# DerrickXuNu/CoBEVT

Measured on AMD Instinct MI355X. Metric: bev_frames_per_sec, higher is better.
Workload: dtype bf16

## Files before the change

cobevt_amd/csrc/stem7x7.hip:

```cpp
#include "common.hpp"
#include "f32_matrix.hpp"

namespace cobevt {

struct StemParams {
    const float* in;
    const unsigned char* in_u8;
    const float* lut;
    const void* wgt;
    const float* bias;
    void* out;
    int N, H, W, Ho, Wo, Cout;
    int act;
    int tiles_y, tiles_x, tiles_n, ntiles;
};

__device__ __forceinline__ uint4 lds_read_2x8(const unsigned char* a) {
    typedef const volatile __attribute__((address_space(3))) unsigned long long* lds_u64_ptr;
    const unsigned long long lo = *(lds_u64_ptr)a, hi = *(lds_u64_ptr)(a + 8);
    return make_uint4((unsigned)lo, (unsigned)(lo >> 32), (unsigned)hi, (unsigned)(hi >> 32));
}

template <typename T> struct StemCfg {
    static constexpr int KB = Elem<T>::kBytes;
    static constexpr int STEPS_ROW = 48 * KB / 32;
    static constexpr int PIX = 12 * KB;
    static constexpr int PH = 11, PW = 19;
    static constexpr int PROW = (PW * PIX - 16 * PIX % 256 + 255) / 256 * 256 + 16 * PIX % 256;
    static constexpr int PATCH = (PH * PROW + 255) / 256 * 256;
    static constexpr int WROW = 192 * KB + 16;
    static constexpr int WBYTES = 64 * WROW;
    static constexpr int SROW = 64 * 4 + 16;
    static constexpr int STAGE = 128 * SROW;
    static constexpr int LDS = PATCH + WBYTES + STAGE;
};

template <typename T>
__global__ __launch_bounds__(256) void stem7x7_kernel(StemParams p) {
    using C = StemCfg<T>;
    constexpr int KB = C::KB;
    constexpr int NPIECE = C::PH * C::PW * 2 * 3;
    constexpr int P_IT = (NPIECE + 255) / 256;
    extern __shared__ __attribute__((aligned(16))) unsigned char smem[];
    unsigned char* patch = smem;
    unsigned char* wl = smem + C::PATCH;
    float* stage = (float*)(smem + C::PATCH + C::WBYTES);

    const int tid = threadIdx.x, lane = tid & 63, wave = tid >> 6;
    const int h = lane >> 5, ql = lane & 31;

    for (int i = tid; i < C::PATCH / 16; i += 256) ((uint4*)patch)[i] = make_uint4(0, 0, 0, 0);

    float2 preg[P_IT];
    auto decode = [&](int tile, int& img, int& oy0, int& ox0, int& n0) {
        const int tn = tile % p.tiles_n;
        int rest = tile / p.tiles_n;
        const int tx = rest % p.tiles_x; rest /= p.tiles_x;
        const int ty = rest % p.tiles_y;
        img = rest / p.tiles_y;
        oy0 = ty * 8; ox0 = tx * 16; n0 = tn * 64;
    };
    auto load_patch = [&](int tile) {
        int img, oy0, ox0, n0;
        decode(tile, img, oy0, ox0, n0);
#pragma unroll
        for (int it = 0; it < P_IT; ++it) {
            const int item = tid + it * 256;
            float2 v = make_float2(0.f, 0.f);
            if (item < NPIECE) {
                const int pc = item % 3, rest = item / 3;
                const int dy = rest & 1, pix = rest >> 1;
                const int py = pix / C::PW, px = pix - py * C::PW;
                const int iy = 2 * (oy0 - 2 + py) + dy, ix = 2 * (ox0 - 2 + px);
                if (iy >= 0 && iy < p.H && ix >= 0 && ix + 1 < p.W)
                    v = *(const float2*)(p.in + (((size_t)img * p.H + iy) * p.W + ix) * 3 + pc * 2);
            }
            preg[it] = v;
        }
    };
    auto store_patch = [&]() {
#pragma unroll
        for (int it = 0; it < P_IT; ++it) {
            const int item = tid + it * 256;
            if (item < NPIECE) {
                const int pc = item % 3, rest = item / 3;
                const int dy = rest & 1, pix = rest >> 1;
                const int py = pix / C::PW, px = pix - py * C::PW;
                unsigned char* dst = patch + py * C::PROW + px * C::PIX + (dy * 6 + pc * 2) * KB;
                if constexpr (Elem<T>::kIsBf16) *(uint32_t*)dst = pack_bf2(preg[it].x, preg[it].y);
                else *(float2*)dst = preg[it];
            }
        }
    };

    int img, oy0, ox0, n0;
    int tile = blockIdx.x;
    if (tile >= p.ntiles) return;
    decode(tile, img, oy0, ox0, n0);
    int n0_loaded = -1;
    auto load_weights = [&](int nb) {
        constexpr int PIECES = 16 * 16 * Elem<T>::kBytes / 16;
        constexpr int PPT = PIECES / 16;
        for (int i = tid; i < 64 * PIECES; i += 256) {
            const int row = i / PIECES, j = i - row * PIECES;
            const int tap = j / PPT, part = j - tap * PPT;
            uint4 v = make_uint4(0, 0, 0, 0);
            if (nb + row < p.Cout) v = *(const uint4*)((const unsigned char*)p.wgt + ((size_t)(nb + row) * PIECES + j) * 16);
            unsigned char* d = wl + row * C::WROW + ((tap >> 2) * 48 + (tap & 3) * 12) * KB + part * 16;
            if constexpr (Elem<T>::kIsBf16) {
                *(uint2*)d = make_uint2(v.x, v.y);
                if (part == 0) *(uint2*)(d + 8) = make_uint2(v.z, v.w);
            } else if (part < 3) {
                *(uint4*)d = v;
            }
        }
        n0_loaded = nb;
    };
    __syncthreads();
    load_patch(tile);
    load_weights(n0);

    const int abase = ((2 * wave + (ql >> 4)) * C::PROW) + (ql & 15) * C::PIX + h * 16;
    const int bbase = ql * C::WROW + h * 16;

    for (; tile < p.ntiles; tile += gridDim.x) {
        decode(tile, img, oy0, ox0, n0);
        store_patch();
        if (n0 != n0_loaded) { __syncthreads(); load_weights(n0); }
        __syncthreads();
        const int next = tile + gridDim.x;
        if (next < p.ntiles) load_patch(next);

        f32x16 acc[2];
#pragma unroll
        for (int b = 0; b < 2; ++b)
#pragma unroll
            for (int r = 0; r < 16; ++r) acc[b][r] = 0.f;
#pragma unroll
        for (int a = 0; a < 4; ++a) {
#pragma unroll
            for (int sub = 0; sub < C::STEPS_ROW; ++sub) {
                const unsigned char* pa = patch + abase + a * C::PROW + sub * 32;
                const unsigned char* pw = wl + bbase + a * 48 * KB + sub * 32;
                uint4 af;
                if constexpr (Elem<T>::kIsBf16) {
                    af = lds_read_2x8(pa);
                } else {
                    af = *(const uint4*)pa;
                }
                const uint4 b0 = *(const uint4*)pw;
                const uint4 b1 = *(const uint4*)(pw + 32 * C::WROW);
                mfma_kgroup<T, false>(af, b0, acc[0]);
                mfma_kgroup<T, false>(af, b1, acc[1]);
            }
        }
        constexpr int SR = C::SROW / 4;
#pragma unroll
        for (int b = 0; b < 2; ++b) {
            const int cl = b * 32 + ql;
            const float bias = (p.bias && n0 + cl < p.Cout) ? p.bias[n0 + cl] : 0.f;
#pragma unroll
            for (int r = 0; r < 16; ++r) {
                const int row = acc_row(r, lane);
                float v = acc[b][r] + bias;
                v = p.act == 1 ? fmaxf(v, 0.f) : v;
                stage[((2 * wave + (row >> 4)) * 16 + (row & 15)) * SR + cl] = v;
            }
        }
        __syncthreads();
        constexpr int CH = Elem<T>::kChunk;
        constexpr int CPP = 64 / CH;
        T* out = (T*)p.out;
        for (int item = tid; item < 128 * CPP; item += 256) {
            const int px = item / CPP, cj = item - px * CPP;
            const int oy = oy0 + (px >> 4), ox = ox0 + (px & 15), col = n0 + cj * CH;
            if (oy >= p.Ho || ox >= p.Wo || col >= p.Cout) continue;
            float v[8];
#pragma unroll
            for (int e = 0; e < CH; ++e) v[e] = stage[px * SR + cj * CH + e];
            const size_t o = (((size_t)img * p.Ho + oy) * p.Wo + ox) * p.Cout + col;
            if (col + CH <= p.Cout) *(uint4*)(out + o) = f32_to_chunk<T>(v);
            else for (int e = 0; e < CH && col + e < p.Cout; ++e) store_elem<T>(out, o + e, v[e]);
        }
        __syncthreads();
    }
}


#ifndef COBEVT_STEM_POOL_ROWS_BF16
#define COBEVT_STEM_POOL_ROWS_BF16 5
#endif
#ifndef COBEVT_STEM_POOL_ROWS_F32
#define COBEVT_STEM_POOL_ROWS_F32 3
#endif
#ifndef COBEVT_STEM_KNOCK
#define COBEVT_STEM_KNOCK 0
#endif

typedef short short2_t __attribute__((ext_vector_type(2)));
template <typename T> __device__ __forceinline__ uint32_t word_max(uint32_t a, uint32_t b) {
    if constexpr (Elem<T>::kIsBf16) {
        const short2_t r = __builtin_elementwise_max(__builtin_bit_cast(short2_t, a), __builtin_bit_cast(short2_t, b));
        return __builtin_bit_cast(uint32_t, r);
    } else {
        return (uint32_t)max((int)a, (int)b);
    }
}

template <typename T> struct StemPoolCfg {
    static constexpr int KB = Elem<T>::kBytes;
    static constexpr int STEPS_ROW = 48 * KB / 32;
    static constexpr int NS = 4 * STEPS_ROW;
    static constexpr int PIX = 12 * KB;
    static constexpr int ROWS = Elem<T>::kIsBf16 ? COBEVT_STEM_POOL_ROWS_BF16 : COBEVT_STEM_POOL_ROWS_F32;
    static constexpr int RH = 2 * ROWS + 1, RW = 17, RPIX = RH * RW;
    static constexpr int NPT = (RPIX + 31) / 32;
    static constexpr int NT = 64 * NPT * 2;
    static constexpr int PH = RH + 3, PW = RW + 3;
    static constexpr int PROW = (PW * PIX - RW * PIX % 256 + 255) / 256 * 256 + RW * PIX % 256;
    static constexpr int PATCH = (PH * PROW + 255) / 256 * 256;
    static constexpr int WROW = 192 * KB + 16;
    static constexpr int WBYTES = 64 * WROW;
    static constexpr int SROW = 64 * Elem<T>::kBytes + 16;
    static constexpr int STAGE = (RPIX * SROW + 255) / 256 * 256;
    static constexpr int LDS = PATCH + WBYTES + STAGE + 256;
    static constexpr int LDS_U8 = LDS + 3 * 256 * 4;
    static_assert(NT <= 1024, "stem_pool_kernel: region too large for one workgroup");
};

#ifdef COBEVT_STEM_TRACE
__device__ unsigned long long cobevt_stem_trace[16];
#define COBEVT_ST_MARK(i) do { if (blockIdx.x == 0 && threadIdx.x == 0 && tile == (int)blockIdx.x + 2 * (int)gridDim.x) cobevt_stem_trace[(i)] = __builtin_readcyclecounter(); } while (0)
#else
#define COBEVT_ST_MARK(i) do {} while (0)
#endif

template <typename T, bool U8 = false>
__global__ __launch_bounds__(StemPoolCfg<T>::NT) void stem_pool_kernel(StemParams p) {
    using C = StemPoolCfg<T>;
    constexpr int RW = C::RW, RPIX = C::RPIX, NT = C::NT, KB = C::KB;
    constexpr int NPIECE = C::PH * C::PW * 2 * 3;
    constexpr int P_IT = (NPIECE + NT - 1) / NT;
    extern __shared__ __attribute__((aligned(16))) unsigned char smem[];
    unsigned char* patch = smem;
    unsigned char* wl = smem + C::PATCH;
    unsigned char* stage = smem + C::PATCH + C::WBYTES;

    const int tid = threadIdx.x, lane = tid & 63, wave = tid >> 6;
    const int h = lane >> 5, ql = lane & 31;
    const int Hp = p.Ho / 2, Wp = p.Wo / 2;

    for (int i = tid; i < C::PATCH / 16; i += NT) ((uint4*)patch)[i] = make_uint4(0, 0, 0, 0);

    int pdst[P_IT], prow[P_IT], pxo[P_IT], pcol[P_IT];
    int plut[P_IT];
#pragma unroll
    for (int it = 0; it < P_IT; ++it) {
        const int item = tid + it * NT;
        pdst[it] = -1; prow[it] = 0; pxo[it] = 0; pcol[it] = 0; plut[it] = 0;
        if (item < NPIECE) {
            const int pc = item % 3, rest = item / 3;
            const int dy = rest & 1, pix = rest >> 1;
            const int py = pix / C::PW, px = pix - py * C::PW;
            pdst[it] = py * C::PROW + px * C::PIX + (dy * 6 + pc * 2) * KB;
            prow[it] = 2 * (py - 2) + dy;
            pxo[it] = 2 * (px - 2);
            pcol[it] = pxo[it] * 3 + pc * 2;
            plut[it] = ((pc * 2) % 3) | (((pc * 2 + 1) % 3) << 8);
        }
    }
    int poff[P_IT];
#pragma unroll
    for (int it = 0; it < P_IT; ++it) poff[it] = prow[it] * p.W * 3 + pcol[it];
    float2 preg[P_IT];
    unsigned int praw[P_IT];
    const float* lut_l = (const float*)(smem + C::LDS);
    auto decode = [&](int tile, int& img, int& py0, int& px0) {
        const int tx = tile % p.tiles_x;
        const int rest = tile / p.tiles_x;
        const int ty = rest % p.tiles_y;
        img = rest / p.tiles_y;
        py0 = ty * C::ROWS; px0 = tx * 8;
    };
    auto load_patch = [&](int tile) {
        int img, py0, px0;
        decode(tile, img, py0, px0);
        const int oy0 = 2 * py0 - 1, ox0 = 2 * px0 - 1;
        const size_t origin = ((size_t)img * p.H + 2 * oy0) * (size_t)p.W * 3 + 6 * ox0;
        const float* base = p.in + origin;
        const unsigned char* base8 = p.in_u8 + origin;
        const int ylo = -2 * oy0, yhi = p.H - 2 * oy0, xlo = -2 * ox0, xhi = p.W - 1 - 2 * ox0;
#pragma unroll
        for (int it = 0; it < P_IT; ++it) {
            const bool ok = (pdst[it] >= 0) & (prow[it] >= ylo) & (prow[it] < yhi) & (pxo[it] >= xlo) & (pxo[it] < xhi);
            if constexpr (U8) {
                unsigned int r = 0x10000u;
                if (!(COBEVT_STEM_KNOCK & 8) && ok) r = *(const unsigned short*)(base8 + poff[it]);
                praw[it] = r;
            } else {
                float2 v = make_float2(0.f, 0.f);
                if (!(COBEVT_STEM_KNOCK & 8) && ok) v = *(const float2*)(base + poff[it]);
                preg[it] = v;
            }
        }
    };
    auto store_patch = [&]() {
        if constexpr (U8) {
#pragma unroll
            for (int it = 0; it < P_IT; ++it) {
                const unsigned int r = praw[it];
                const float a = lut_l[(plut[it] & 0xff) * 256 + (r & 0xff)], b = lut_l[(plut[it] >> 8) * 256 + ((r >> 8) & 0xff)];
                preg[it] = (r >> 16) ? make_float2(0.f, 0.f) : make_float2(a, b);
            }
        }
#pragma unroll
        for (int it = 0; it < P_IT; ++it)
            if (pdst[it] >= 0) {
                unsigned char* dst = patch + pdst[it];
                if constexpr (Elem<T>::kIsBf16) *(uint32_t*)dst = pack_bf2(preg[it].x, preg[it].y);
                else if constexpr (kXSplit<T>) {
                    uint32_t hi, lo;
                    split_pair_staged(preg[it].x, preg[it].y, hi, lo);
                    unsigned char* pb = patch + (pdst[it] & ~15) + ((pdst[it] >> 1) & 4);
                    *(uint32_t*)pb = hi;
                    *(uint32_t*)(pb + 8) = lo;
                } else *(float2*)dst = preg[it];
            }
    };

    int tile = blockIdx.x;
    if (tile >= p.ntiles) return;
    if constexpr (U8) {
        float* l = (float*)(smem + C::LDS);
        for (int i = tid; i < 768; i += NT) l[i] = p.lut[i];
    }
    {
        load_patch(tile);
        constexpr int PIECES = 16 * 16 * KB / 16;
        constexpr int PPT = PIECES / 16;
        constexpr int W_IT = (64 * PIECES + NT - 1) / NT;
        uint4 wv[W_IT];
#pragma unroll
        for (int it = 0; it < W_IT; ++it) {
            const int i = tid + it * NT;
            const int row = i / PIECES, j = i - row * PIECES;
            wv[it] = *(const uint4*)((const unsigned char*)p.wgt + ((size_t)(row < p.Cout ? row : 0) * PIECES + (i < 64 * PIECES ? j : 0)) * 16);
        }
#pragma unroll
        for (int it = 0; it < W_IT; ++it) {
            const int i = tid + it * NT;
            const int row = i / PIECES, j = i - row * PIECES;
            const int tap = j / PPT, part = j - tap * PPT;
            if (i < 64 * PIECES) {
                const uint4 v = row < p.Cout ? wv[it] : make_uint4(0, 0, 0, 0);
                unsigned char* d = wl + row * C::WROW + ((tap >> 2) * 48 + (tap & 3) * 12) * KB + part * 16;
                if constexpr (Elem<T>::kIsBf16) {
                    *(uint2*)d = make_uint2(v.x, v.y);
                    if (part == 0) *(uint2*)(d + 8) = make_uint2(v.z, v.w);
                } else if (part < 3) {
                    *(uint4*)d = stage_w_piece<T>(v);
                }
            }
        }
    }

    const int chalf = wave & 1;
    const int rpix = (wave >> 1) * 32 + ql;
    const int rpc = rpix < RPIX ? rpix : RPIX - 1;
    const int ry = rpc / RW, rx = rpc - ry * RW;
    const int abase = ry * C::PROW + rx * C::PIX + h * 16;
    const int bbase = (chalf * 32 + ql) * C::WROW + h * 16;
    float* bias_l = (float*)(smem + C::PATCH + C::WBYTES + C::STAGE);
    if (tid < 64) bias_l[tid] = p.bias ? p.bias[tid] : 0.f;
    __syncthreads();

    constexpr int CH = Elem<T>::kChunk;
    constexpr int CPP = 64 / CH;
    static_assert((C::ROWS + 1) / 2 * 2 * 8 * CPP <= NT, "stem_pool_kernel: one pooled chunk per thread (rows in pairs)");
    uint4 pend = make_uint4(0, 0, 0, 0);
    T* pend_dst = nullptr;

    for (; tile < p.ntiles; tile += gridDim.x) {
        int img, py0, px0;
        decode(tile, img, py0, px0);
        const int oy0 = 2 * py0 - 1, ox0 = 2 * px0 - 1;
        COBEVT_ST_MARK(0);
        store_patch();
        if (pend_dst) *(uint4*)pend_dst = pend;
        __syncthreads();
        COBEVT_ST_MARK(1);
        const int next = tile + gridDim.x;
        if (next < p.ntiles) load_patch(next);
        COBEVT_ST_MARK(2);

        f32x16 acc;
#pragma unroll
        for (int r = 0; r < 16; ++r) acc[r] = 0.f;
        constexpr int NS = C::NS;
        constexpr int RS = 2;
        uint4 ra[RS], rb[RS];
        auto fetch = [&](int slot, int i) {
            const int a = i / C::STEPS_ROW, sub = i - a * C::STEPS_ROW;
            rb[slot] = *(const uint4*)(wl + bbase + a * 48 * KB + sub * 32);
            const unsigned char* pa = patch + abase + a * C::PROW + sub * 32;
            if constexpr (Elem<T>::kIsBf16) {
                ra[slot] = lds_read_2x8(pa);
            } else {
                ra[slot] = *(const uint4*)pa;
            }
        };
#pragma unroll
        for (int i = 0; i < RS - 1; ++i) fetch(i, i);
        __builtin_amdgcn_sched_barrier(0);
#pragma unroll
        for (int i = 0; i < NS; ++i) {
            if (i + RS - 1 < NS && !(COBEVT_STEM_KNOCK & 1)) fetch((i + RS - 1) % RS, i + RS - 1);
            if constexpr (COBEVT_STEM_KNOCK & 2) asm volatile("" :: "v"(rb[i % RS].x), "v"(rb[i % RS].y), "v"(rb[i % RS].z), "v"(rb[i % RS].w), "v"(ra[i % RS].x), "v"(ra[i % RS].y), "v"(ra[i % RS].z), "v"(ra[i % RS].w));
            else
            mfma_kgroup_staged<T>(rb[i % RS], ra[i % RS], acc);
            __builtin_amdgcn_sched_barrier(0);
        }
        COBEVT_ST_MARK(3);
        if (rpix < RPIX && !(COBEVT_STEM_KNOCK & 16)) {
            const int oy = oy0 + ry, ox = ox0 + rx;
            const bool inside = oy >= 0 && oy < p.Ho && ox >= 0 && ox < p.Wo;
            float4 bq[4];
#pragma unroll
            for (int k = 0; k < 4; ++k) bq[k] = *(const float4*)(bias_l + chalf * 32 + 8 * k + 4 * h);
            __builtin_amdgcn_sched_barrier(0);
#pragma unroll
            for (int k = 0; k < 4; ++k) {
                const int c0 = chalf * 32 + 8 * k + 4 * h;
                const float4 b = bq[k];
                float v[4] = {acc[4 * k] + b.x, acc[4 * k + 1] + b.y, acc[4 * k + 2] + b.z, acc[4 * k + 3] + b.w};
#pragma unroll
                for (int e = 0; e < 4; ++e) v[e] = inside ? fmaxf(v[e], 0.f) : 0.f;
                unsigned char* d = stage + rpix * C::SROW + c0 * Elem<T>::kBytes;
                if constexpr (Elem<T>::kIsBf16) *(uint2*)d = make_uint2(pack_bf2(v[0], v[1]), pack_bf2(v[2], v[3]));
                else *(float4*)d = make_float4(v[0], v[1], v[2], v[3]);
            }
        }
        COBEVT_ST_MARK(4);
        __syncthreads();
        COBEVT_ST_MARK(5);
        pend_dst = nullptr;
        int q_y, q_x, cj;
        if constexpr (Elem<T>::kIsBf16) {
            const int hw = tid >> 5, j = (tid >> 3) & 3, t = hw & 3;
            q_y = 2 * (hw >> 2) + (j & 1);
            q_x = j == 0 ? t : j == 1 ? ((t + 7) & 7) : j == 2 ? t + 4 : t + 3;
            cj = tid & 7;
        } else {
            const int q = tid / CPP;
            q_y = q >> 3; q_x = q & 7; cj = tid - q * CPP;
        }
        if (q_y < C::ROWS) {
            const int qy = q_y, qx = q_x;
            const int py = py0 + qy, px = px0 + qx;
            uint4 wv[9];
#pragma unroll
            for (int dy = 0; dy < 3; ++dy)
#pragma unroll
                for (int dx = 0; dx < 3; ++dx) {
                    wv[dy * 3 + dx] = *(const uint4*)(stage + ((2 * qy + dy) * RW + 2 * qx + dx) * C::SROW + cj * 16);
                    if constexpr (COBEVT_STEM_KNOCK & 4) wv[dy * 3 + dx] = make_uint4(dy, dx, dy, dx);
                }
            __builtin_amdgcn_sched_barrier(0);
            uint4 m = make_uint4(0, 0, 0, 0);
#pragma unroll
            for (int i = 0; i < 9; ++i) {
                m.x = word_max<T>(m.x, wv[i].x); m.y = word_max<T>(m.y, wv[i].y);
                m.z = word_max<T>(m.z, wv[i].z); m.w = word_max<T>(m.w, wv[i].w);
            }
            pend = m;
            if (py < Hp && px < Wp) pend_dst = (T*)p.out + (((size_t)img * Hp + py) * Wp + px) * 64 + cj * CH;
        }
        COBEVT_ST_MARK(6);
        __syncthreads();
        COBEVT_ST_MARK(7);
    }
    if (pend_dst) *(uint4*)pend_dst = pend;
}

}

using namespace cobevt;

extern "C" int cobevt_stem_conv7x7s2(const float* in, const void* wgt, const float* bias, void* out, const int* dims,
                                     hipStream_t stream) {
    if (!in || !wgt || !out || !dims) return COBEVT_ERR_ARG;
    StemParams p;
    const int dtype = dims[0];
    p.in = in; p.in_u8 = nullptr; p.lut = nullptr; p.wgt = wgt; p.bias = bias; p.out = out;
    p.N = dims[1]; p.H = dims[2]; p.W = dims[3]; p.Cout = dims[4]; p.act = dims[5];
    if (dtype != 0 && dtype != 1) return COBEVT_ERR_ARG;
    if (p.N < 1 || p.H < 2 || p.W < 2 || (p.H & 1) || (p.W & 1) || p.Cout < 1) return COBEVT_ERR_SHAPE;
    if (p.Cout % (dtype == 0 ? 8 : 4)) return COBEVT_ERR_SHAPE;
    p.Ho = p.H / 2; p.Wo = p.W / 2;
    p.tiles_y = (p.Ho + 7) / 8; p.tiles_x = (p.Wo + 15) / 16; p.tiles_n = (p.Cout + 63) / 64;
    const long nt = (long)p.N * p.tiles_y * p.tiles_x * p.tiles_n;
    if (nt > 0x7fffffffL) return COBEVT_ERR_SHAPE;
    p.ntiles = (int)nt;
    const size_t lds = dtype == 0 ? StemCfg<bf16_t>::LDS : StemCfg<float>::LDS;
    cobevt::allow_dynamic_lds<stem7x7_kernel<bf16_t>>((int)StemCfg<bf16_t>::LDS);
    cobevt::allow_dynamic_lds<stem7x7_kernel<float>>((int)StemCfg<float>::LDS);
    const int per_cu = dtype == 0 ? 2 : 1;
    const unsigned blocks = (unsigned)(nt < 256L * per_cu ? nt : 256L * per_cu);
    if (dtype == 0) hipLaunchKernelGGL(stem7x7_kernel<bf16_t>, dim3(blocks), dim3(256), lds, stream, p);
    else hipLaunchKernelGGL(stem7x7_kernel<float>, dim3(blocks), dim3(256), lds, stream, p);
    return cobevt::launch_status();
}

extern "C" int cobevt_stem_conv7x7s2_pool(const float* in, const void* wgt, const float* bias, void* out, const int* dims,
                                          hipStream_t stream) {
    if (!in || !wgt || !out || !dims) return COBEVT_ERR_ARG;
    StemParams p;
    const int dtype = dims[0];
    p.in = in; p.in_u8 = nullptr; p.lut = nullptr; p.wgt = wgt; p.bias = bias; p.out = out;
    p.N = dims[1]; p.H = dims[2]; p.W = dims[3]; p.Cout = 64; p.act = 1;
    if (dtype != 0 && dtype != 1) return COBEVT_ERR_ARG;
    if (p.N < 1 || p.H < 4 || p.W < 4 || (p.H & 3) || (p.W & 3)) return COBEVT_ERR_SHAPE;
    p.Ho = p.H / 2; p.Wo = p.W / 2;
    const int rows = dtype == 0 ? StemPoolCfg<bf16_t>::ROWS : StemPoolCfg<float>::ROWS;
    p.tiles_y = (p.Ho / 2 + rows - 1) / rows; p.tiles_x = (p.Wo / 2 + 7) / 8; p.tiles_n = 1;
    const long nt = (long)p.N * p.tiles_y * p.tiles_x;
    if (nt > 0x7fffffffL) return COBEVT_ERR_SHAPE;
    p.ntiles = (int)nt;
    const size_t lds = dtype == 0 ? StemPoolCfg<bf16_t>::LDS : StemPoolCfg<float>::LDS;
    cobevt::allow_dynamic_lds<stem_pool_kernel<bf16_t>>((int)StemPoolCfg<bf16_t>::LDS);
    cobevt::allow_dynamic_lds<stem_pool_kernel<float>>((int)StemPoolCfg<float>::LDS);
    const int nthreads = dtype == 0 ? StemPoolCfg<bf16_t>::NT : StemPoolCfg<float>::NT;
    int per_cu = (int)(163840 / lds);
    if (per_cu > 2048 / nthreads) per_cu = 2048 / nthreads;
    if (per_cu < 1) per_cu = 1;
    const unsigned blocks = (unsigned)(nt < 256L * per_cu ? nt : 256L * per_cu);
    if (dtype == 0) hipLaunchKernelGGL(stem_pool_kernel<bf16_t>, dim3(blocks), dim3(StemPoolCfg<bf16_t>::NT), lds, stream, p);
    else hipLaunchKernelGGL(stem_pool_kernel<float>, dim3(blocks), dim3(StemPoolCfg<float>::NT), lds, stream, p);
    return cobevt::launch_status();
}

extern "C" int cobevt_stem_conv7x7s2_pool_u8(const unsigned char* in, const float* lut, const void* wgt, const float* bias, void* out,
                                             const int* dims, hipStream_t stream) {
    if (!in || !lut || !wgt || !out || !dims) return COBEVT_ERR_ARG;
    StemParams p;
    const int dtype = dims[0];
    p.in = nullptr; p.in_u8 = in; p.lut = lut; p.wgt = wgt; p.bias = bias; p.out = out;
    p.N = dims[1]; p.H = dims[2]; p.W = dims[3]; p.Cout = 64; p.act = 1;
    if (dtype != 0 && dtype != 1) return COBEVT_ERR_ARG;
    if (p.N < 1 || p.H < 4 || p.W < 4 || (p.H & 3) || (p.W & 3)) return COBEVT_ERR_SHAPE;
    p.Ho = p.H / 2; p.Wo = p.W / 2;
    const int rows = dtype == 0 ? StemPoolCfg<bf16_t>::ROWS : StemPoolCfg<float>::ROWS;
    p.tiles_y = (p.Ho / 2 + rows - 1) / rows; p.tiles_x = (p.Wo / 2 + 7) / 8; p.tiles_n = 1;
    const long nt = (long)p.N * p.tiles_y * p.tiles_x;
    if (nt > 0x7fffffffL) return COBEVT_ERR_SHAPE;
    p.ntiles = (int)nt;
    const size_t lds = dtype == 0 ? StemPoolCfg<bf16_t>::LDS_U8 : StemPoolCfg<float>::LDS_U8;
    cobevt::allow_dynamic_lds<stem_pool_kernel<bf16_t, true>>((int)StemPoolCfg<bf16_t>::LDS_U8);
    cobevt::allow_dynamic_lds<stem_pool_kernel<float, true>>((int)StemPoolCfg<float>::LDS_U8);
    const int nthreads = dtype == 0 ? StemPoolCfg<bf16_t>::NT : StemPoolCfg<float>::NT;
    int per_cu = (int)(163840 / lds);
    if (per_cu > 2048 / nthreads) per_cu = 2048 / nthreads;
    if (per_cu < 1) per_cu = 1;
    const unsigned blocks = (unsigned)(nt < 256L * per_cu ? nt : 256L * per_cu);
    if (dtype == 0) hipLaunchKernelGGL((stem_pool_kernel<bf16_t, true>), dim3(blocks), dim3(StemPoolCfg<bf16_t>::NT), lds, stream, p);
    else hipLaunchKernelGGL((stem_pool_kernel<float, true>), dim3(blocks), dim3(StemPoolCfg<float>::NT), lds, stream, p);
    return cobevt::launch_status();
}

#ifdef COBEVT_STEM_TRACE
extern "C" int cobevt_stem_read_trace(unsigned long long* dst) {
    return hipMemcpyFromSymbol(dst, HIP_SYMBOL(cobevt_stem_trace), sizeof(unsigned long long) * 16) == hipSuccess ? 0 : 1;
}
#endif
```

Before: 622.0.

## Keep stem conv weights in registers, two pixels per wave, packed piece descriptors

For bf16, the fused 7x7 stem conv + maxpool kernel now holds its weights in VGPRs instead of LDS. That frees the weight LDS region and allows taller tiles (7 pooled rows) and two workgroups per CU. Each wave computes two pixel groups against one 32-channel half, so every weight register is reused across pixels. Patch-load descriptors are packed into one int per piece, and interior tiles skip the bounds checks. Register pressure rises sharply, with launch bounds of 4 waves/EU, which risks spills and fewer waves in flight; an optional XCD-aware tile split is added but disabled.

```diff
diff --git a/cobevt_amd/csrc/stem7x7.hip b/cobevt_amd/csrc/stem7x7.hip
--- a/cobevt_amd/csrc/stem7x7.hip
+++ b/cobevt_amd/csrc/stem7x7.hip
@@ -1,3 +1,4 @@
+#include <type_traits>
 #include "common.hpp"
 #include "f32_matrix.hpp"
 
@@ -187,14 +188,26 @@
 }
 
 
+#ifndef COBEVT_STEM_LAYOUT
+#define COBEVT_STEM_LAYOUT 2
+#endif
 #ifndef COBEVT_STEM_POOL_ROWS_BF16
-#define COBEVT_STEM_POOL_ROWS_BF16 5
+#define COBEVT_STEM_POOL_ROWS_BF16 (COBEVT_STEM_LAYOUT == 2 ? 7 : 5)
 #endif
 #ifndef COBEVT_STEM_POOL_ROWS_F32
 #define COBEVT_STEM_POOL_ROWS_F32 3
 #endif
 #ifndef COBEVT_STEM_KNOCK
 #define COBEVT_STEM_KNOCK 0
+#endif
+#ifndef COBEVT_STEM_WAVES_EU
+#define COBEVT_STEM_WAVES_EU (COBEVT_STEM_LAYOUT == 2 ? 4 : 2)
+#endif
+#ifndef COBEVT_STEM_PER_CU
+#define COBEVT_STEM_PER_CU (COBEVT_STEM_LAYOUT == 2 ? 2 : 1)
+#endif
+#ifndef COBEVT_STEM_XCD
+#define COBEVT_STEM_XCD 0
 #endif
 
 typedef short short2_t __attribute__((ext_vector_type(2)));
@@ -215,28 +228,44 @@
     static constexpr int ROWS = Elem<T>::kIsBf16 ? COBEVT_STEM_POOL_ROWS_BF16 : COBEVT_STEM_POOL_ROWS_F32;
     static constexpr int RH = 2 * ROWS + 1, RW = 17, RPIX = RH * RW;
     static constexpr int NPT = (RPIX + 31) / 32;
-    static constexpr int NT = 64 * NPT * 2;
+    static constexpr int LAYOUT = Elem<T>::kIsBf16 ? COBEVT_STEM_LAYOUT : 0;
+    static constexpr bool REGW = LAYOUT != 0;
+    static constexpr int NPX = LAYOUT == 2 ? 2 : 1;
+    static constexpr int NCH = LAYOUT == 1 ? 2 : 1;
+    static constexpr int NWAVE = (NPT + NPX - 1) / NPX * (2 / NCH);
+    static constexpr int NT = 64 * NWAVE;
     static constexpr int PH = RH + 3, PW = RW + 3;
     static constexpr int PROW = (PW * PIX - RW * PIX % 256 + 255) / 256 * 256 + RW * PIX % 256;
     static constexpr int PATCH = (PH * PROW + 255) / 256 * 256;
     static constexpr int WROW = 192 * KB + 16;
-    static constexpr int WBYTES = 64 * WROW;
+    static constexpr int WBYTES = REGW ? 0 : 64 * WROW;
     static constexpr int SROW = 64 * Elem<T>::kBytes + 16;
     static constexpr int STAGE = (RPIX * SROW + 255) / 256 * 256;
     static constexpr int LDS = PATCH + WBYTES + STAGE + 256;
     static constexpr int LDS_U8 = LDS + 3 * 256 * 4;
     static_assert(NT <= 1024, "stem_pool_kernel: region too large for one workgroup");
+    static constexpr int WAVES_EU = REGW ? COBEVT_STEM_WAVES_EU : 1;
+    static constexpr int REG_WG = REGW ? COBEVT_STEM_PER_CU : 8;
+    static unsigned grid(long ntiles, size_t lds) {
+        int per_cu = (int)(163840 / lds);
+        if (per_cu > 2048 / NT) per_cu = 2048 / NT;
+        if (per_cu > REG_WG) per_cu = REG_WG;
+        if (per_cu < 1) per_cu = 1;
+        return (unsigned)(ntiles < 256L * per_cu ? ntiles : 256L * per_cu);
+    }
 };
 
 #ifdef COBEVT_STEM_TRACE
 __device__ unsigned long long cobevt_stem_trace[16];
-#define COBEVT_ST_MARK(i) do { if (blockIdx.x == 0 && threadIdx.x == 0 && tile == (int)blockIdx.x + 2 * (int)gridDim.x) cobevt_stem_trace[(i)] = __builtin_readcyclecounter(); } while (0)
+#define COBEVT_ST_MARK(i) do { if (blockIdx.x == 0 && threadIdx.x == 0 && tile_no == ((i) < 8 ? 2 : 0)) cobevt_stem_trace[(i)] = __builtin_readcyclecounter(); } while (0)
+#define COBEVT_ST_MARK_ENDS(i) do { if (blockIdx.x == 0 && threadIdx.x == 0) cobevt_stem_trace[(i)] = (i) == 13 ? (unsigned long long)tile_no : __builtin_readcyclecounter(); } while (0)
 #else
 #define COBEVT_ST_MARK(i) do {} while (0)
+#define COBEVT_ST_MARK_ENDS(i) do {} while (0)
 #endif
 
 template <typename T, bool U8 = false>
-__global__ __launch_bounds__(StemPoolCfg<T>::NT) void stem_pool_kernel(StemParams p) {
+__global__ __launch_bounds__(StemPoolCfg<T>::NT, StemPoolCfg<T>::WAVES_EU) void stem_pool_kernel(StemParams p) {
     using C = StemPoolCfg<T>;
     constexpr int RW = C::RW, RPIX = C::RPIX, NT = C::NT, KB = C::KB;
     constexpr int NPIECE = C::PH * C::PW * 2 * 3;
@@ -252,26 +281,28 @@
 
     for (int i = tid; i < C::PATCH / 16; i += NT) ((uint4*)patch)[i] = make_uint4(0, 0, 0, 0);
 
-    int pdst[P_IT], prow[P_IT], pxo[P_IT], pcol[P_IT];
-    int plut[P_IT];
+    static_assert(C::PATCH <= 0x4000 && 2 * C::PH + 8 < 64 && 6 * C::PW < 256, "stem_pool_kernel: packed piece word");
+    int pdesc[P_IT];
 #pragma unroll
     for (int it = 0; it < P_IT; ++it) {
         const int item = tid + it * NT;
-        pdst[it] = -1; prow[it] = 0; pxo[it] = 0; pcol[it] = 0; plut[it] = 0;
+        pdesc[it] = -1;
         if (item < NPIECE) {
             const int pc = item % 3, rest = item / 3;
             const int dy = rest & 1, pix = rest >> 1;
             const int py = pix / C::PW, px = pix - py * C::PW;
-            pdst[it] = py * C::PROW + px * C::PIX + (dy * 6 + pc * 2) * KB;
-            prow[it] = 2 * (py - 2) + dy;
-            pxo[it] = 2 * (px - 2);
-            pcol[it] = pxo[it] * 3 + pc * 2;
-            plut[it] = ((pc * 2) % 3) | (((pc * 2 + 1) % 3) << 8);
-        }
-    }
-    int poff[P_IT];
-#pragma unroll
-    for (int it = 0; it < P_IT; ++it) poff[it] = prow[it] * p.W * 3 + pcol[it];
+            pdesc[it] = (py * C::PROW + px * C::PIX + (dy * 6 + pc * 2) * KB) | ((2 * (py - 2) + dy + 8) << 14) | ((6 * px + 2 * pc) << 20) | (pc << 28);
+        }
+    }
+    auto piece = [&](int it) {
+        int d = pdesc[it];
+        if constexpr (C::REGW) asm volatile("" : "+v"(d));
+        return d;
+    };
+    auto piece_dst = [](int d) { return d & 0x3fff; };
+    auto piece_row = [](int d) { return (d >> 14) & 63; };
+    auto piece_col = [](int d) { return (d >> 20) & 255; };
+    auto piece_pc = [](int d) { return (d >> 28) & 3; };
     float2 preg[P_IT];
     unsigned int praw[P_IT];
     const float* lut_l = (const float*)(smem + C::LDS);
@@ -286,55 +317,96 @@
         int img, py0, px0;
         decode(tile, img, py0, px0);
         const int oy0 = 2 * py0 - 1, ox0 = 2 * px0 - 1;
-        const size_t origin = ((size_t)img * p.H + 2 * oy0) * (size_t)p.W * 3 + 6 * ox0;
+        const int w3 = p.W * 3;
+        const long long origin = ((long long)img * p.H + 2 * oy0 - 8) * (long long)w3 + 6 * ox0 - 12;
         const float* base = p.in + origin;
         const unsigned char* base8 = p.in_u8 + origin;
-        const int ylo = -2 * oy0, yhi = p.H - 2 * oy0, xlo = -2 * ox0, xhi = p.W - 1 - 2 * ox0;
-#pragma unroll
-        for (int it = 0; it < P_IT; ++it) {
-            const bool ok = (pdst[it] >= 0) & (prow[it] >= ylo) & (prow[it] < yhi) & (pxo[it] >= xlo) & (pxo[it] < xhi);
-            if constexpr (U8) {
-                unsigned int r = 0x10000u;
-                if (!(COBEVT_STEM_KNOCK & 8) && ok) r = *(const unsigned short*)(base8 + poff[it]);
-                praw[it] = r;
-            } else {
-                float2 v = make_float2(0.f, 0.f);
-                if (!(COBEVT_STEM_KNOCK & 8) && ok) v = *(const float2*)(base + poff[it]);
-                preg[it] = v;
-            }
-        }
+        const int rlo = 8 - 2 * oy0, rhi = p.H + 8 - 2 * oy0, clo = 6 * (2 - ox0), chi = 6 * (p.W / 2 + 2 - ox0);
+        const bool interior = rlo <= 4 && rhi > 2 * C::PH + 3 && clo <= 0 && chi >= 6 * C::PW;
+        auto issue = [&](auto checked) {
+#pragma unroll
+            for (int it = 0; it < P_IT; ++it) {
+                const int d = piece(it), row = piece_row(d), col = piece_col(d);
+                bool ok = d >= 0;
+                if constexpr (decltype(checked)::value) ok = ok & (row >= rlo) & (row < rhi) & (col >= clo) & (col < chi);
+                const int poff = row * w3 + col;
+                if constexpr (U8) {
+                    unsigned int r = 0x10000u;
+                    if (!(COBEVT_STEM_KNOCK & 8) && ok) r = *(const unsigned short*)(base8 + poff);
+                    praw[it] = r;
+                } else {
+                    float2 v = make_float2(0.f, 0.f);
+                    if (!(COBEVT_STEM_KNOCK & 8) && ok) v = *(const float2*)(base + poff);
+                    preg[it] = v;
+                }
+            }
+        };
+        if (interior) issue(std::false_type()); else issue(std::true_type());
     };
     auto store_patch = [&]() {
         if constexpr (U8) {
 #pragma unroll
             for (int it = 0; it < P_IT; ++it) {
                 const unsigned int r = praw[it];
-                const float a = lut_l[(plut[it] & 0xff) * 256 + (r & 0xff)], b = lut_l[(plut[it] >> 8) * 256 + ((r >> 8) & 0xff)];
+                const int pc = piece_pc(piece(it));
+                const int c0 = pc == 0 ? 0 : 3 - pc, c1 = pc == 1 ? 0 : c0 + 1;
+                const float a = lut_l[c0 * 256 + (r & 0xff)], b = lut_l[c1 * 256 + ((r >> 8) & 0xff)];
                 preg[it] = (r >> 16) ? make_float2(0.f, 0.f) : make_float2(a, b);
             }
         }
 #pragma unroll
         for (int it = 0; it < P_IT; ++it)
-            if (pdst[it] >= 0) {
-                unsigned char* dst = patch + pdst[it];
+            if (pdesc[it] >= 0) {
+                const int pdst = piece_dst(piece(it));
+                unsigned char* dst = patch + pdst;
                 if constexpr (Elem<T>::kIsBf16) *(uint32_t*)dst = pack_bf2(preg[it].x, preg[it].y);
                 else if constexpr (kXSplit<T>) {
                     uint32_t hi, lo;
                     split_pair_staged(preg[it].x, preg[it].y, hi, lo);
-                    unsigned char* pb = patch + (pdst[it] & ~15) + ((pdst[it] >> 1) & 4);
+                    unsigned char* pb = patch + (pdst & ~15) + ((pdst >> 1) & 4);
                     *(uint32_t*)pb = hi;
                     *(uint32_t*)(pb + 8) = lo;
                 } else *(float2*)dst = preg[it];
             }
     };
 
-    int tile = blockIdx.x;
-    if (tile >= p.ntiles) return;
+    int tile = blockIdx.x, tstep = gridDim.x, tend = p.ntiles;
+    if constexpr (COBEVT_STEM_XCD) {
+        const int nblk = gridDim.x, xcd = blockIdx.x & 7, slot = blockIdx.x >> 3;
+        const int q = nblk >> 3, r = nblk & 7;
+        const int first = xcd < r ? xcd * (q + 1) : r * (q + 1) + (xcd - r) * q;
+        tstep = q + (xcd < r);
+        tile = (int)((long long)p.ntiles * first / nblk) + slot;
+        tend = (int)((long long)p.ntiles * (first + tstep) / nblk);
+    }
+    if (tile >= tend) return;
+    [[maybe_unused]] int tile_no = 0;
+    COBEVT_ST_MARK_ENDS(11);
     if constexpr (U8) {
         float* l = (float*)(smem + C::LDS);
         for (int i = tid; i < 768; i += NT) l[i] = p.lut[i];
     }
-    {
+    const int chalf0 = C::NCH == 2 ? 0 : (wave & 1);
+    const int ptile0 = C::NCH == 2 ? wave : (wave >> 1) * C::NPX;
+    uint4 breg[C::REGW ? C::NCH : 1][C::REGW ? C::NS : 1];
+    if constexpr (C::REGW) {
+        static_assert(Elem<T>::kIsBf16, "stem_pool_kernel: register-resident weights are the bf16 form");
+        load_patch(tile);
+        COBEVT_ST_MARK(8);
+#pragma unroll
+        for (int c = 0; c < C::NCH; ++c) {
+            const unsigned char* wrow = (const unsigned char*)p.wgt + (size_t)((chalf0 + c) * 32 + ql) * 512;
+#pragma unroll
+            for (int i = 0; i < C::NS; ++i) {
+                const int a = i / C::STEPS_ROW, sub = i - a * C::STEPS_ROW;
+                const int g0 = 4 * sub + 2 * h, g1 = g0 + 1;
+                const uint2 lo = *(const uint2*)(wrow + (a * 4 + g0 / 3) * 32 + (g0 % 3) * 8);
+                const uint2 hi = *(const uint2*)(wrow + (a * 4 + g1 / 3) * 32 + (g1 % 3) * 8);
+                breg[c][i] = make_uint4(lo.x, lo.y, hi.x, hi.y);
+            }
+        }
+        COBEVT_ST_MARK(9);
+    } else {
         load_patch(tile);
         constexpr int PIECES = 16 * 16 * KB / 16;
         constexpr int PPT = PIECES / 16;
@@ -364,45 +436,61 @@
         }
     }
 
-    const int chalf = wave & 1;
-    const int rpix = (wave >> 1) * 32 + ql;
-    const int rpc = rpix < RPIX ? rpix : RPIX - 1;
-    const int ry = rpc / RW, rx = rpc - ry * RW;
-    const int abase = ry * C::PROW + rx * C::PIX + h * 16;
-    const int bbase = (chalf * 32 + ql) * C::WROW + h * 16;
+    auto region_pixel = [&](int u, int& rpix, int& ry, int& rx) {
+        rpix = (ptile0 + u) * 32 + ql;
+        const int rpc = rpix < RPIX ? rpix : RPIX - 1;
+        ry = rpc / RW; rx = rpc - ry * RW;
+    };
+    int abase[C::NPX];
+#pragma unroll
+    for (int u = 0; u < C::NPX; ++u) {
+        int rpix, ry, rx;
+        region_pixel(u, rpix, ry, rx);
+        abase[u] = ry * C::PROW + rx * C::PIX + h * 16;
+    }
+    [[maybe_unused]] const int bbase = (chalf0 * 32 + ql) * C::WROW + h * 16;
     float* bias_l = (float*)(smem + C::PATCH + C::WBYTES + C::STAGE);
     if (tid < 64) bias_l[tid] = p.bias ? p.bias[tid] : 0.f;
     __syncthreads();
+    COBEVT_ST_MARK(10);
 
     constexpr int CH = Elem<T>::kChunk;
     constexpr int CPP = 64 / CH;
     static_assert((C::ROWS + 1) / 2 * 2 * 8 * CPP <= NT, "stem_pool_kernel: one pooled chunk per thread (rows in pairs)");
     uint4 pend = make_uint4(0, 0, 0, 0);
-    T* pend_dst = nullptr;
-
-    for (; tile < p.ntiles; tile += gridDim.x) {
+    constexpr unsigned NO_PEND = 0xffffffffu;
+    unsigned pend_chunk = NO_PEND;
+
+    for (; tile < tend; tile += tstep, ++tile_no) {
         int img, py0, px0;
         decode(tile, img, py0, px0);
         const int oy0 = 2 * py0 - 1, ox0 = 2 * px0 - 1;
         COBEVT_ST_MARK(0);
         store_patch();
-        if (pend_dst) *(uint4*)pend_dst = pend;
+        if (pend_chunk != NO_PEND) ((uint4*)p.out)[pend_chunk] = pend;
         __syncthreads();
         COBEVT_ST_MARK(1);
-        const int next = tile + gridDim.x;
-        if (next < p.ntiles) load_patch(next);
+        const int next = tile + tstep;
+        if (next < tend) load_patch(next);
         COBEVT_ST_MARK(2);
 
-        f32x16 acc;
-#pragma unroll
-        for (int r = 0; r < 16; ++r) acc[r] = 0.f;
+        f32x16 acc[C::NPX][C::NCH];
+#pragma unroll
+        for (int u = 0; u < C::NPX; ++u)
+#pragma unroll
+            for (int c = 0; c < C::NCH; ++c)
+#pragma unroll
+                for (int r = 0; r < 16; ++r) acc[u][c][r] = 0.f;
         constexpr int NS = C::NS;
         constexpr int RS = 2;
-        uint4 ra[RS], rb[RS];
-        auto fetch = [&](int slot, int i) {
+        constexpr int NF = NS * C::NPX;
+        uint4 ra[RS];
+        [[maybe_unused]] uint4 rb[RS];
+        auto fetch = [&](int slot, int s) {
+            const int i = s / C::NPX, u = s - i * C::NPX;
             const int a = i / C::STEPS_ROW, sub = i - a * C::STEPS_ROW;
-            rb[slot] = *(const uint4*)(wl + bbase + a * 48 * KB + sub * 32);
-            const unsigned char* pa = patch + abase + a * C::PROW + sub * 32;
+            if constexpr (!C::REGW) rb[slot] = *(const uint4*)(wl + bbase + a * 48 * KB + sub * 32);
+            const unsigned char* pa = patch + abase[u] + a * C::PROW + sub * 32;
             if constexpr (Elem<T>::kIsBf16) {
                 ra[slot] = lds_read_2x8(pa);
             } else {
@@ -410,40 +498,58 @@
             }
         };
 #pragma unroll
-        for (int i = 0; i < RS - 1; ++i) fetch(i, i);
+        for (int s = 0; s < RS - 1; ++s) fetch(s, s);
         __builtin_amdgcn_sched_barrier(0);
 #pragma unroll
-        for (int i = 0; i < NS; ++i) {
-            if (i + RS - 1 < NS && !(COBEVT_STEM_KNOCK & 1)) fetch((i + RS - 1) % RS, i + RS - 1);
-            if constexpr (COBEVT_STEM_KNOCK & 2) asm volatile("" :: "v"(rb[i % RS].x), "v"(rb[i % RS].y), "v"(rb[i % RS].z), "v"(rb[i % RS].w), "v"(ra[i % RS].x), "v"(ra[i % RS].y), "v"(ra[i % RS].z), "v"(ra[i % RS].w));
-            else
-            mfma_kgroup_staged<T>(rb[i % RS], ra[i % RS], acc);
+        for (int s = 0; s < NF; ++s) {
+            if (s + RS - 1 < NF && !(COBEVT_STEM_KNOCK & 1)) fetch((s + RS - 1) % RS, s + RS - 1);
+            const int i = s / C::NPX, u = s - i * C::NPX;
+#pragma unroll
+            for (int c = 0; c < C::NCH; ++c) {
+                const uint4& wv = C::REGW ? breg[c][C::REGW ? i : 0] : rb[s % RS];
+                const uint4& xv = ra[s % RS];
+                if constexpr (COBEVT_STEM_KNOCK & 2) asm volatile("" :: "v"(wv.x), "v"(wv.y), "v"(wv.z), "v"(wv.w), "v"(xv.x), "v"(xv.y), "v"(xv.z), "v"(xv.w));
+                else mfma_kgroup_staged<T>(wv, xv, acc[u][c]);
+            }
             __builtin_amdgcn_sched_barrier(0);
         }
         COBEVT_ST_MARK(3);
-        if (rpix < RPIX && !(COBEVT_STEM_KNOCK & 16)) {
-            const int oy = oy0 + ry, ox = ox0 + rx;
-            const bool inside = oy >= 0 && oy < p.Ho && ox >= 0 && ox < p.Wo;
-            float4 bq[4];
-#pragma unroll
-            for (int k = 0; k < 4; ++k) bq[k] = *(const float4*)(bias_l + chalf * 32 + 8 * k + 4 * h);
-            __builtin_amdgcn_sched_barrier(0);
-#pragma unroll
-            for (int k = 0; k < 4; ++k) {
-                const int c0 = chalf * 32 + 8 * k + 4 * h;
-                const float4 b = bq[k];
-                float v[4] = {acc[4 * k] + b.x, acc[4 * k + 1] + b.y, acc[4 * k + 2] + b.z, acc[4 * k + 3] + b.w};
-#pragma unroll
-                for (int e = 0; e < 4; ++e) v[e] = inside ? fmaxf(v[e], 0.f) : 0.f;
-                unsigned char* d = stage + rpix * C::SROW + c0 * Elem<T>::kBytes;
-                if constexpr (Elem<T>::kIsBf16) *(uint2*)d = make_uint2(pack_bf2(v[0], v[1]), pack_bf2(v[2], v[3]));
-                else *(float4*)d = make_float4(v[0], v[1], v[2], v[3]);
+#pragma unroll
+        for (int u = 0; u < C::NPX; ++u) {
+            int rpix, ry, rx;
+            region_pixel(u, rpix, ry, rx);
+            if (rpix < RPIX && !(COBEVT_STEM_KNOCK & 16)) {
+                const int oy = oy0 + ry, ox = ox0 + rx;
+                const bool inside = oy >= 0 && oy < p.Ho && ox >= 0 && ox < p.Wo;
+                constexpr int BQ = C::REGW ? 2 : 4;
+#pragma unroll
+                for (int c = 0; c < C::NCH; ++c)
+#pragma unroll
+                    for (int k0 = 0; k0 < 4; k0 += BQ) {
+                        float4 bq[BQ];
+#pragma unroll
+                        for (int k = 0; k < BQ; ++k) bq[k] = *(const float4*)(bias_l + (chalf0 + c) * 32 + 8 * (k0 + k) + 4 * h);
+                        __builtin_amdgcn_sched_barrier(0);
+#pragma unroll
+                        for (int kk = 0; kk < BQ; ++kk) {
+                            const int k = k0 + kk;
+                            const int c0 = (chalf0 + c) * 32 + 8 * k + 4 * h;
+                            const float4 b = bq[kk];
+                            const f32x16& ac = acc[u][c];
+                            float v[4] = {ac[4 * k] + b.x, ac[4 * k + 1] + b.y, ac[4 * k + 2] + b.z, ac[4 * k + 3] + b.w};
+#pragma unroll
+                            for (int e = 0; e < 4; ++e) v[e] = inside ? fmaxf(v[e], 0.f) : 0.f;
+                            unsigned char* d = stage + rpix * C::SROW + c0 * Elem<T>::kBytes;
+                            if constexpr (Elem<T>::kIsBf16) *(uint2*)d = make_uint2(pack_bf2(v[0], v[1]), pack_bf2(v[2], v[3]));
+                            else *(float4*)d = make_float4(v[0], v[1], v[2], v[3]);
+                        }
+                    }
             }
         }
         COBEVT_ST_MARK(4);
         __syncthreads();
         COBEVT_ST_MARK(5);
-        pend_dst = nullptr;
+        pend_chunk = NO_PEND;
         int q_y, q_x, cj;
         if constexpr (Elem<T>::kIsBf16) {
             const int hw = tid >> 5, j = (tid >> 3) & 3, t = hw & 3;
@@ -457,29 +563,35 @@
         if (q_y < C::ROWS) {
             const int qy = q_y, qx = q_x;
             const int py = py0 + qy, px = px0 + qx;
-            uint4 wv[9];
-#pragma unroll
-            for (int dy = 0; dy < 3; ++dy)
-#pragma unroll
-                for (int dx = 0; dx < 3; ++dx) {
-                    wv[dy * 3 + dx] = *(const uint4*)(stage + ((2 * qy + dy) * RW + 2 * qx + dx) * C::SROW + cj * 16);
-                    if constexpr (COBEVT_STEM_KNOCK & 4) wv[dy * 3 + dx] = make_uint4(dy, dx, dy, dx);
+            constexpr int WB = C::LAYOUT == 1 ? 1 : 3;
+            uint4 m = make_uint4(0, 0, 0, 0);
+#pragma unroll
+            for (int dy0 = 0; dy0 < 3; dy0 += WB) {
+                uint4 wv[WB * 3];
+#pragma unroll
+                for (int dy = 0; dy < WB; ++dy)
+#pragma unroll
+                    for (int dx = 0; dx < 3; ++dx) {
+                        wv[dy * 3 + dx] = *(const uint4*)(stage + ((2 * qy + dy0 + dy) * RW + 2 * qx + dx) * C::SROW + cj * 16);
+                        if constexpr (COBEVT_STEM_KNOCK & 4) wv[dy * 3 + dx] = make_uint4(dy0 + dy, dx, dy0 + dy, dx);
+                    }
+                __builtin_amdgcn_sched_barrier(0);
+#pragma unroll
+                for (int i = 0; i < WB * 3; ++i) {
+                    m.x = word_max<T>(m.x, wv[i].x); m.y = word_max<T>(m.y, wv[i].y);
+                    m.z = word_max<T>(m.z, wv[i].z); m.w = word_max<T>(m.w, wv[i].w);
                 }
-            __builtin_amdgcn_sched_barrier(0);
-            uint4 m = make_uint4(0, 0, 0, 0);
-#pragma unroll
-            for (int i = 0; i < 9; ++i) {
-                m.x = word_max<T>(m.x, wv[i].x); m.y = word_max<T>(m.y, wv[i].y);
-                m.z = word_max<T>(m.z, wv[i].z); m.w = word_max<T>(m.w, wv[i].w);
             }
             pend = m;
-            if (py < Hp && px < Wp) pend_dst = (T*)p.out + (((size_t)img * Hp + py) * Wp + px) * 64 + cj * CH;
+            if (py < Hp && px < Wp) pend_chunk = ((unsigned)(img * Hp + py) * Wp + px) * CPP + cj;
         }
         COBEVT_ST_MARK(6);
         __syncthreads();
         COBEVT_ST_MARK(7);
     }
-    if (pend_dst) *(uint4*)pend_dst = pend;
+    if (pend_chunk != NO_PEND) ((uint4*)p.out)[pend_chunk] = pend;
+    COBEVT_ST_MARK_ENDS(12);
+    COBEVT_ST_MARK_ENDS(13);
 }
 
 }
@@ -525,15 +637,12 @@
     p.tiles_y = (p.Ho / 2 + rows - 1) / rows; p.tiles_x = (p.Wo / 2 + 7) / 8; p.tiles_n = 1;
     const long nt = (long)p.N * p.tiles_y * p.tiles_x;
     if (nt > 0x7fffffffL) return COBEVT_ERR_SHAPE;
+    if ((long)p.N * (p.Ho / 2) * (p.Wo / 2) * 16 >= 0xffffffffL) return COBEVT_ERR_SHAPE;
     p.ntiles = (int)nt;
     const size_t lds = dtype == 0 ? StemPoolCfg<bf16_t>::LDS : StemPoolCfg<float>::LDS;
     cobevt::allow_dynamic_lds<stem_pool_kernel<bf16_t>>((int)StemPoolCfg<bf16_t>::LDS);
     cobevt::allow_dynamic_lds<stem_pool_kernel<float>>((int)StemPoolCfg<float>::LDS);
-    const int nthreads = dtype == 0 ? StemPoolCfg<bf16_t>::NT : StemPoolCfg<float>::NT;
-    int per_cu = (int)(163840 / lds);
-    if (per_cu > 2048 / nthreads) per_cu = 2048 / nthreads;
-    if (per_cu < 1) per_cu = 1;
-    const unsigned blocks = (unsigned)(nt < 256L * per_cu ? nt : 256L * per_cu);
+    const unsigned blocks = dtype == 0 ? StemPoolCfg<bf16_t>::grid(nt, lds) : StemPoolCfg<float>::grid(nt, lds);
     if (dtype == 0) hipLaunchKernelGGL(stem_pool_kernel<bf16_t>, dim3(blocks), dim3(StemPoolCfg<bf16_t>::NT), lds, stream, p);
     else hipLaunchKernelGGL(stem_pool_kernel<float>, dim3(blocks), dim3(StemPoolCfg<float>::NT), lds, stream, p);
     return cobevt::launch_status();
@@ -553,15 +662,12 @@
     p.tiles_y = (p.Ho / 2 + rows - 1) / rows; p.tiles_x = (p.Wo / 2 + 7) / 8; p.tiles_n = 1;
     const long nt = (long)p.N * p.tiles_y * p.tiles_x;
     if (nt > 0x7fffffffL) return COBEVT_ERR_SHAPE;
+    if ((long)p.N * (p.Ho / 2) * (p.Wo / 2) * 16 >= 0xffffffffL) return COBEVT_ERR_SHAPE;
     p.ntiles = (int)nt;
     const size_t lds = dtype == 0 ? StemPoolCfg<bf16_t>::LDS_U8 : StemPoolCfg<float>::LDS_U8;
     cobevt::allow_dynamic_lds<stem_pool_kernel<bf16_t, true>>((int)StemPoolCfg<bf16_t>::LDS_U8);
     cobevt::allow_dynamic_lds<stem_pool_kernel<float, true>>((int)StemPoolCfg<float>::LDS_U8);
-    const int nthreads = dtype == 0 ? StemPoolCfg<bf16_t>::NT : StemPoolCfg<float>::NT;
-    int per_cu = (int)(163840 / lds);
-    if (per_cu > 2048 / nthreads) per_cu = 2048 / nthreads;
-    if (per_cu < 1) per_cu = 1;
-    const unsigned blocks = (unsigned)(nt < 256L * per_cu ? nt : 256L * per_cu);
+    const unsigned blocks = dtype == 0 ? StemPoolCfg<bf16_t>::grid(nt, lds) : StemPoolCfg<float>::grid(nt, lds);
     if (dtype == 0) hipLaunchKernelGGL((stem_pool_kernel<bf16_t, true>), dim3(blocks), dim3(StemPoolCfg<bf16_t>::NT), lds, stream, p);
     else hipLaunchKernelGGL((stem_pool_kernel<float, true>), dim3(blocks), dim3(StemPoolCfg<float>::NT), lds, stream, p);
     return cobevt::launch_status();
```

After: 621.3. Within noise of the previous version (-0.1%).
